# apple/ml-neuman

Measured on NVIDIA H100. Metric: Mrays/sec @128+128 samples, higher is better.
Workload: dtype f16 operands x f32 accumulate (wgmma); f32 elsewhere

## Files before the change

neuman_b200/csrc/api.cu:

```cuda
#include <math.h>
#include <string.h>

#include "nm_internal.cuh"

extern "C" const char* nm_version(void) { return "neuman_b200 0.1 (sm_90a)"; }

extern "C" int nm_ctx_create(int device, nm_ctx** out) {
  if (!out) return NM_ERR_INVALID;
  *out = nullptr;
  int ndev = 0;
  if (cudaGetDeviceCount(&ndev) != cudaSuccess || device < 0 || device >= ndev) return NM_ERR_CUDA;
  if (cudaSetDevice(device) != cudaSuccess) return NM_ERR_CUDA;
  nm_ctx* c = new nm_ctx();
  c->device = device;
  cudaDeviceProp prop;
  if (cudaGetDeviceProperties(&prop, device) == cudaSuccess) c->sm_count = prop.multiProcessorCount;
  if (cudaMalloc(&c->d_counter, 64 * sizeof(int32_t)) != cudaSuccess ||
      cudaMallocHost(&c->h_counter, 64 * sizeof(int32_t)) != cudaSuccess) {
    delete c;
    return NM_ERR_CUDA;
  }
  cudaMemset(c->d_counter, 0, 64 * sizeof(int32_t));
  *out = c;
  return NM_OK;
// ... 267 lines not shown
  const int rc = check_view_desc(ctx, d, __func__);
  if (rc != NM_OK) return rc;
  return net_pack(ctx, slot, d, NM_NET_NERFT, nullptr, nullptr, (cudaStream_t)stream);
}

extern "C" int nm_net_pack_noview(nm_ctx* ctx, int slot, const nm_nerf_noview_desc* d, void* stream) {
  NM_ENTER(ctx);
  if (slot < 0 || slot >= NM_MAX_NET_SLOTS || !d) NM_FAIL(ctx, NM_ERR_INVALID, "nm_net_pack_noview: bad slot/desc");
  if (d->pos_n_freqs != 10)
    NM_FAIL(ctx, NM_ERR_UNSUPPORTED, "nm_net_pack_noview: only pos_N_freqs=10 (63-d encoding) is built");
  for (int l = 0; l < 8; ++l)
    if (!d->pts_w[l] || !d->pts_b[l]) NM_FAIL(ctx, NM_ERR_INVALID, "nm_net_pack_noview: null pts_linears");
  if (!d->output_w || !d->output_b) NM_FAIL(ctx, NM_ERR_INVALID, "nm_net_pack_noview: null output_linear");
  nm_nerf_desc full{};
  for (int l = 0; l < 8; ++l) { full.pts_w[l] = d->pts_w[l]; full.pts_b[l] = d->pts_b[l]; }
  full.pos_pe_kind = d->pos_pe_kind;
  full.pos_min_freq = d->pos_min_freq; full.pos_max_freq = d->pos_max_freq; full.pos_n_freqs = d->pos_n_freqs;
  full.dir_pe_kind = NM_PE_POSENC; full.dir_min_freq = 0.f; full.dir_max_freq = 3.f; full.dir_n_freqs = 4;
  return net_pack(ctx, slot, &full, NM_NET_NOVIEW, d->output_w, d->output_b, (cudaStream_t)stream);
}

static int mlp_dispatch(nm_ctx* ctx, int slot, int mode, const float* pts, const float* views, const float* origins,
                        const float* dirs, const float* z, int64_t n, int32_t group, float t, float* raw, void* stream,
                        const NmTrainStash* stash = nullptr) {
  if (slot < 0 || slot >= NM_MAX_NET_SLOTS || !ctx->nets[slot].packed)
    NM_FAIL(ctx, NM_ERR_STATE, "nm_mlp_forward: net slot not packed");
  if (n < 0 || !raw) NM_FAIL(ctx, NM_ERR_INVALID, "nm_mlp_forward: bad argument");
  if (n == 0) return NM_OK;
  NmNet& net = ctx->nets[slot];
  if (mode != NM_MLP_SIMT_F32 && mode != NM_MLP_TC_F16) NM_FAIL(ctx, NM_ERR_INVALID, "nm_mlp_forward: unknown mode");
  cudaStream_t st = (cudaStream_t)stream;
  cudaEvent_t e0 = nullptr, e1 = nullptr;
  if (ctx->profile) {
    if (ctx->prof_used + 2 > ctx->prof_events.size()) {
      for (int k = 0; k < 2; ++k) {
        cudaEvent_t e;
        NM_CHECK_CUDA(ctx, cudaEventCreate(&e));
        ctx->prof_events.push_back(e);
      }
    }
    e0 = ctx->prof_events[ctx->prof_used];
    e1 = ctx->prof_events[ctx->prof_used + 1];
    NM_CHECK_CUDA(ctx, cudaEventRecord(e0, st));
  }
  int rc = mode == NM_MLP_SIMT_F32 ? nm_simt_forward(ctx, net, pts, views, origins, dirs, z, n, group, t, raw, st)
                                   : nm_tc_forward(ctx, net, pts, views, origins, dirs, z, n, group, t, raw, st, stash);
  if (ctx->profile && rc == NM_OK) {
    NM_CHECK_CUDA(ctx, cudaEventRecord(e1, st));
    ctx->prof_used += 2;
    ctx->prof_evals += n;
  }
  return rc;
}

static bool views_ok(const nm_ctx* ctx, int slot, const void* views) {
  return views || (slot >= 0 && slot < NM_MAX_NET_SLOTS && ctx->nets[slot].packed && ctx->nets[slot].kind == NM_NET_NOVIEW);
}
static bool is_noview(const nm_ctx* ctx, int slot) {
  return slot >= 0 && slot < NM_MAX_NET_SLOTS && ctx->nets[slot].kind == NM_NET_NOVIEW;
}
static bool is_nerft(const nm_ctx* ctx, int slot) {
  return slot >= 0 && slot < NM_MAX_NET_SLOTS && ctx->nets[slot].packed && ctx->nets[slot].kind == NM_NET_NERFT;
}

extern "C" int nm_mlp_forward(nm_ctx* ctx, int slot, int mode, const float* pts, const float* views, int64_t n,
                              int32_t views_per_ray, float* raw, void* stream) {
  NM_ENTER(ctx);
  if (!pts || !views_ok(ctx, slot, views) || views_per_ray < 0) NM_FAIL(ctx, NM_ERR_INVALID, "nm_mlp_forward: null pts/views");
  if (views_per_ray > 0 && n % views_per_ray != 0)
// ... 56 lines not shown
  const int width = 3 + 6 * (which == 0 ? net.desc.pos_n_freqs : net.desc.dir_n_freqs);
  if (ld < width) NM_FAIL(ctx, NM_ERR_INVALID, "nm_pe_backward: ld smaller than the encoding width");
  if (n == 0) return NM_OK;
  if (!x || !d_enc || !d_x) NM_FAIL(ctx, NM_ERR_INVALID, "nm_pe_backward: null argument");
  return nm_impl_pe_backward(ctx, net, which, x, group, d_enc, ld, inv_scale, n, d_x, (cudaStream_t)stream);
}

extern "C" int nm_dw_gemm(nm_ctx* ctx, const void* g_pre, const void* g_f, const void* g_v, const void* stash_x,
                          const void* stash_f, int64_t n, float* out, float* bias_out, void* stream) {
  NM_ENTER(ctx);
  if (n < 0 || !out || !bias_out) NM_FAIL(ctx, NM_ERR_INVALID, "nm_dw_gemm: bad argument");
  if (n == 0) {
    NM_CHECK_CUDA(ctx, cudaMemsetAsync(out, 0, (size_t)9 * 256 * 256 * sizeof(float), (cudaStream_t)stream));
    NM_CHECK_CUDA(ctx, cudaMemsetAsync(bias_out, 0, (size_t)9 * 256 * sizeof(float), (cudaStream_t)stream));
    return NM_OK;
  }
  const bool trunk_only = !g_f && !g_v && !stash_f;
  if (!g_pre || !stash_x || (!trunk_only && (!g_f || !g_v || !stash_f))) NM_FAIL(ctx, NM_ERR_INVALID, "nm_dw_gemm: null argument");
  return nm_impl_dw_gemm(ctx, (const __half*)g_pre, (const __half*)g_f, (const __half*)g_v, (const __half*)stash_x,
                         (const __half*)stash_f, n, out, bias_out, (cudaStream_t)stream);
}

int nm_impl_mlp_forward_rays(nm_ctx* ctx, int slot, int mode, const float* origins, const float* dirs, const float* z,
                             int64_t R, int32_t S, float t, float* raw, cudaStream_t st) {
  if (!origins || !dirs || !z || S <= 0 || R < 0) NM_FAIL(ctx, NM_ERR_INVALID, "nm_mlp_forward_rays: bad argument");
  return mlp_dispatch(ctx, slot, mode, nullptr, nullptr, origins, dirs, z, R * (int64_t)S, S, t, raw, st);
}

extern "C" int nm_mlp_forward_rays(nm_ctx* ctx, int slot, int mode, const float* origins, const float* dirs,
                                   const float* z, int64_t R, int32_t S, float* raw, void* stream) {
  NM_ENTER(ctx);
  if (is_nerft(ctx, slot)) NM_FAIL(ctx, NM_ERR_UNSUPPORTED, "nm_mlp_forward_rays: a NeRF-T net needs the time (nm_render_vanilla_t)");
  return nm_impl_mlp_forward_rays(ctx, slot, mode, origins, dirs, z, R, S, 0.f, raw, (cudaStream_t)stream);
}
```

neuman_b200/csrc/mlp_tc.cu:

```cuda
#include "nm_internal.cuh"
#include "nm_pe.cuh"
#include "tc_common.cuh"
#include <string.h>
#define TC_MAX_SLABS 64
struct TcPlan {
  uint32_t slab_off[TC_STEPS][6];
  uint32_t slab_bytes[TC_STEPS];
  uint32_t image_bytes;
  uint32_t lin_off[TC_MAX_SLABS + 1];
};

__host__ __device__ constexpr int tc_steps(bool v) { return v ? TC_STEPS : 9; }
__host__ __device__ constexpr int step_nkb(int s, bool v = true, bool t = false) {
  return s == 0 ? (t ? 2 : 1) : (s == 10 ? 2 : (!v && s == 8 ? 4 : (t && s == 5 ? 6 : 5)));
}
__host__ __device__ constexpr bool kb_is_bias(int s, int kb, bool v = true) {
  return kb == 4 && s != 5 && s != 9 && s >= 1 && (v ? s <= 8 : s <= 7);
}
__host__ __device__ constexpr bool kb_is_time(int s, int kb, bool t) { return t && ((s == 0 && kb == 1) || (s == 5 && kb == 5)); }
__host__ __device__ constexpr int step_N(int s, bool v = true) { return s <= 7 || (v && s == 8) ? 256 : (v && s == 9 ? 128 : 16); }
__host__ __device__ constexpr bool kb_is_dir(int s, int kb, bool v = true) { return v && s == 9 && kb == 4; }
__host__ __device__ constexpr int tc_slabs_per_tile(bool v = true, bool t = false) {
  int n = 0;
  for (int s = 0; s < tc_steps(v); ++s) n += step_nkb(s, v, t);
  return n;
}
static_assert(tc_slabs_per_tile(true, true) <= TC_MAX_SLABS && tc_slabs_per_tile(true) <= TC_MAX_SLABS, "slab table too small");

template <bool kTrain, bool kView>
struct TcCfg {
  static constexpr int THREADS = 256;
  static constexpr int NSLOT = kTrain || kView ? 4 : 6;
  static constexpr int OFF_POS = kTrain ? 4 * TC_KB_BYTES : 0;
  static constexpr int OFF_DIR = OFF_POS + TC_KB_BYTES;
  static constexpr int WG_BYTES = OFF_DIR + TC_KB_BYTES;
  static constexpr int OFF_RING = 2 * WG_BYTES;
  static constexpr int OFF_BAR = OFF_RING + NSLOT * TC_SLAB_BYTES;
  static constexpr int OFF_CONST = OFF_BAR + 16 * NSLOT;
  static constexpr int SMEM_USED = OFF_CONST + 4 * TC_CONST_FLOATS;
  static constexpr int SMEM_BYTES = SMEM_USED + 1024;
};
static_assert(TcCfg<false, false>::SMEM_BYTES <= 232448 && TcCfg<false, true>::SMEM_BYTES <= 232448 &&
              TcCfg<true, false>::SMEM_BYTES <= 232448 && TcCfg<true, true>::SMEM_BYTES <= 232448,
              "shared memory of the forward kernel exceeds 227 KB");

#define TC_CONST_ALPHA 0
#define TC_CONST_OUT 256

struct TcParams {
  const uint8_t* wimg;
  TcPlan plan;
  NmMlpInput in;
  NmPeSpec pos_pe, dir_pe;
  float* raw;
  const float* consts;
  long long n_tiles;
  int32_t* range_flag;
  int range_phase;
  __half* st_x;
  __half* st_f;
  __half* st_v;
  uint32_t* st_m;
  CUtensorMap map_x, map_f, map_v;
};

__device__ __forceinline__ void sincos_cycles(float f, float& s, float& c) {
// ... 42 lines not shown
        }
      }
    }
  }
  ch[nq == 30 ? 63 : 27] = 1.f;
#pragma unroll
  for (int i = 0; i < 32; ++i) out[i] = pack_f16x2(ch[2 * i], ch[2 * i + 1], false);
}

__device__ __forceinline__ void encode_time_f16(const NmPeSpec& pe, float t, uint32_t (&out)[32]) {
  float ch[22];
  ch[0] = t; ch[21] = 0.f;
#pragma unroll
  for (int k = 0; k < 10; ++k) {
    const float fh = __ldg(pe.table + 2 * k), fl = __ldg(pe.table + 2 * k + 1);
    const float pr = t * fh;
    const float low = fmaf(t, fl, fmaf(t, fh, -pr));
    sincos_cycles((pr - rintf(pr)) + low, ch[1 + 2 * k], ch[2 + 2 * k]);
  }
#pragma unroll
  for (int i = 0; i < 11; ++i) out[16 + i] = pack_f16x2(ch[2 * i], ch[2 * i + 1], false);
}

__device__ __forceinline__ void store_row_swizzled(uint8_t* blk, int row, const uint32_t* v, int nchunks) {
#pragma unroll
  for (int j = 0; j < 8; ++j) {
    if (j < nchunks) {
      uint4 q = make_uint4(v[4 * j], v[4 * j + 1], v[4 * j + 2], v[4 * j + 3]);
      *reinterpret_cast<uint4*>(blk + row * 128 + ((j ^ (row & 7)) << 4)) = q;
    }
  }
}

template <bool RELU>
__device__ __forceinline__ uint32_t pack2(float lo, float hi) {
  uint32_t d;
  if (RELU) asm("cvt.rn.satfinite.relu.f16x2.f32 %0, %1, %2;" : "=r"(d) : "f"(hi), "f"(lo));
  else asm("cvt.rn.satfinite.f16x2.f32 %0, %1, %2;" : "=r"(d) : "f"(hi), "f"(lo));
  return d;
}

template <bool RELU>
__device__ __forceinline__ void track_range(uint32_t& rng, uint32_t packed) {
  __half2 h = *reinterpret_cast<const __half2*>(&packed);
  if (!RELU) h = __habs2(h);
  const __half2 m = __hmax2(*reinterpret_cast<const __half2*>(&rng), h);
  rng = *reinterpret_cast<const uint32_t*>(&m);
}

template <int NC, bool RELU, bool ALPHA, bool SIGNS, bool SMEM>
// ... 19 lines not shown
      a[2 * j] = pA;
      a[2 * j + 1] = pB;
    }
    if (track) { track_range<RELU>(rng, pA); track_range<RELU>(rng, pB); }
    if (SIGNS) {
      const __half2 zero2 = __float2half2_rn(0.f);
      const uint32_t mA = __hgt2_mask(*reinterpret_cast<const __half2*>(&pA), zero2);
      const uint32_t mB = __hgt2_mask(*reinterpret_cast<const __half2*>(&pB), zero2);
      const int bit = 16 * ((j >> 1) & 1) + 4 * (j & 1) + q;
      wA[j >> 2] |= ((mA & 1u) << bit) | ((mA >> 16 & 1u) << (bit + 8));
      wB[j >> 2] |= ((mB & 1u) << bit) | ((mB >> 16 & 1u) << (bit + 8));
    }
  }
}

__device__ __forceinline__ void quad_or(uint32_t (&w)[8]) {
#pragma unroll
  for (int i = 0; i < 8; ++i) {
    w[i] |= __shfl_xor_sync(0xffffffffu, w[i], 1);
    w[i] |= __shfl_xor_sync(0xffffffffu, w[i], 2);
  }
}

template <bool kTrain, bool kView, bool kTime = false>
__device__ __forceinline__ void mlp_tc_body(const TcParams& P) {
  static_assert(!kTime || kView, "NeRF-T nets are view-dependent");
  using C = TcCfg<kTrain, kView>;
  constexpr int SLABS = tc_slabs_per_tile(kView, kTime);
  constexpr int STEPS = tc_steps(kView);
  constexpr int LAST = STEPS - 1;
  extern __shared__ uint8_t smem_dyn[];
  const uint32_t pad = (1024 - (smem_u32(smem_dyn) & 1023)) & 1023;
  uint8_t* smem = smem_dyn + pad;
  const uint32_t sbase = smem_u32(smem);
  const int wg = threadIdx.x >> 7, wtid = threadIdx.x & 127;
  const int lane = threadIdx.x & 31, q = lane & 3;
  const int rA = 16 * (wtid >> 5) + (lane >> 2);
  uint8_t* wbuf = smem + wg * C::WG_BYTES;
  const uint32_t wbase = sbase + wg * C::WG_BYTES;
  float* s_const = reinterpret_cast<float*>(smem + C::OFF_CONST);
  const TcRing<C::NSLOT> R{sbase + C::OFF_RING, sbase + C::OFF_BAR};

  for (int i = threadIdx.x; i < TC_CONST_FLOATS; i += C::THREADS) s_const[i] = __ldg(P.consts + i);
  const long long my_tiles = blockIdx.x < P.n_tiles ? (P.n_tiles - 1 - blockIdx.x) / gridDim.x + 1 : 0;
  const uint32_t total = (uint32_t)(my_tiles * SLABS);
  auto fill = [&](uint32_t qq) {
    const uint32_t j = qq % SLABS, off = P.plan.lin_off[j], bytes = P.plan.lin_off[j + 1] - off;
    mbar_arrive_expect_tx(R.full(qq), bytes);
    bulk_g2s(R.slot(qq), P.wimg + off, bytes, R.full(qq));
  };
  if (threadIdx.x == 0) R.init(total, fill);
  __syncthreads();
// ... 8 lines not shown
  for (long long it = 0; it < my_tiles; ++it) {
    const long long tile = blockIdx.x + it * gridDim.x;
    const long long row0 = tile * 128 + wg * TC_WG_ROWS;
    const bool track = !kView || (it % rperiod) == (P.range_phase % rperiod);
    {
      const int r = wtid & 63;
      const int group = P.in.group;
      long long g0 = 0;
      uint32_t g0r = 0;
      if (group > 0) { g0 = tile * 128 / group; g0r = (uint32_t)(tile * 128 - g0 * group); }
      const uint32_t off = wg * TC_WG_ROWS + r;
      const long long g = group > 0 ? g0 + (g0r + off) / (uint32_t)group : row0 + r;
      float p[3] = {0.f, 0.f, 0.f}, v[3] = {0.f, 0.f, 0.f};
      float t = 0.f;
      if (row0 + r < P.in.n) {
        nm_fetch_sample_at<kTime ? 4 : 3>(P.in, row0 + r, g, p, v);
        if (kTime) t = nm_fetch_time(P.in, row0 + r);
      }
      if (!kTrain && it > 0) wg_sync(wg);
      uint32_t e[32];
      if (wtid < 64) {
        encode_f16(P.pos_pe, p, e, 30);
        store_row_swizzled(wbuf + C::OFF_POS, r, e, 8);
      } else if (kView) {
        encode_f16(P.dir_pe, v, e, 12);
        if (kTime) encode_time_f16(P.pos_pe, t, e);
        store_row_swizzled(wbuf + C::OFF_DIR, r, e, kTime ? 8 : 4);
      }
      if (track && (kView || wtid < 64)) { track_range<false>(rng, e[0]); track_range<false>(rng, e[1]); }
      if (kTime && track && wtid >= 64) track_range<false>(rng, e[16]);
      fence_async_smem();
      wg_sync(wg);
    }
    float alpha[2] = {0.f, 0.f};
#pragma unroll (kTrain ? 1 : STEPS)
    for (int s = 0; s < STEPS; ++s) {
      const int nkb = step_nkb(s, kView, kTime);
      const bool wide = s <= (kView ? 8 : 7), views = kView && s == 9;
      wgmma_fence();
      int kb = 0;
      auto kblock = [&](auto&& issue) {
        const uint32_t qq = qbase + kb;
        R.wait_full(qq);
        issue(gmma_desc_k(R.slot(qq)), kb == 0);
        wgmma_commit();
        if (kb > 0) { wgmma_wait<1>(); R.release(qq - 1, total, fill); }
        ++kb;
      };
      auto smem_kblock = [&](uint32_t a_addr, int k0, int k1) {
        kblock([&](uint64_t b_desc, bool first) {
          const uint64_t a_desc = gmma_desc_k(a_addr);
          for (int k = k0; k < k1; ++k) {
            const uint32_t acc = !first || k > k0;
            if (wide) wgmma_n256(d, a_desc + 2 * k, b_desc + 2 * k, acc);
            else if (views) wgmma_n128(d, a_desc + 2 * k, b_desc + 2 * k, acc);
            else wgmma_n16(d16, a_desc + 2 * k, b_desc + 2 * k, acc);
          }
        });
      };
      if (s == 0 || s == 5) smem_kblock(wbase + C::OFF_POS, 0, 4);
      if (s > 0) {
        const int nact = kView && s == LAST ? 2 : 4;
#pragma unroll
        for (int j = 0; j < 4; ++j) {
          if (j < nact) {
            if constexpr (kTrain) smem_kblock(wbase + j * TC_KB_BYTES, 0, 4);
            else kblock([&](uint64_t b_desc, bool first) {
#pragma unroll
              for (int k = 0; k < 4; ++k) {
                const uint32_t* f = a + 16 * j + 4 * k;
                const uint32_t acc = !first || k > 0;
                if (wide) wgmma_n256_rs(d, f[0], f[1], f[2], f[3], b_desc + 2 * k, acc);
                else if (views) wgmma_n128_rs(d, f[0], f[1], f[2], f[3], b_desc + 2 * k, acc);
                else wgmma_n16_rs(d16, f[0], f[1], f[2], f[3], b_desc + 2 * k, acc);
              }
            });
          }
        }
      }
      if (kb < nkb) {
        if (kb_is_bias(s, kb, kView)) smem_kblock(wbase + C::OFF_POS, 3, 4);
        else if (kb_is_dir(s, kb, kView)) smem_kblock(wbase + C::OFF_DIR, 0, 2);
        else smem_kblock(wbase + C::OFF_DIR, 2, 4);
      }
      wgmma_wait<0>();
      wgmma_fence_regs(d);
      wgmma_fence_regs(d16);
      R.release(qbase + nkb - 1, total, fill);
      qbase += nkb;
      if (s < LAST) {
        if (kTrain) {
          if (wtid == 0) tma_store_wait_read();
          wg_sync(wg);
        }
        uint32_t wA[8] = {0, 0, 0, 0, 0, 0, 0, 0}, wB[8] = {0, 0, 0, 0, 0, 0, 0, 0};
        const float* s_walpha = s_const + TC_CONST_ALPHA;
        if (s == 7) fwd_epi<256, true, kView, kTrain, kTrain>(d, a, wbuf, rA, q, s_walpha, alpha, wA, wB, track, rng);
        else if (kView && s == 8) fwd_epi<256, false, false, false, kTrain>(d, a, wbuf, rA, q, s_walpha, alpha, wA, wB, track, rng);
        else if (s == 9) fwd_epi<128, true, false, kTrain, kTrain>(d, a, wbuf, rA, q, s_walpha, alpha, wA, wB, track, rng);
        else fwd_epi<256, true, false, kTrain, kTrain>(d, a, wbuf, rA, q, s_walpha, alpha, wA, wB, track, rng);
        if (kTrain) {
          fence_async_smem();
          wg_sync(wg);
          if (wtid == 0) {
            if (!kView || s < 8) tma_store_rows(&P.map_x, wbase, 0, 4, row0, s);
            else if (s == 8) tma_store_rows(&P.map_f, wbase, 0, 4, row0, 0);
            else tma_store_rows(&P.map_v, wbase, 0, 2, row0, 0);
          }
          if (!kView || s != 8) {
            quad_or(wA);
            quad_or(wB);
            const long long iA = row0 + rA, iB = iA + 8;
            if (!kView || s < 8) {
              uint32_t* m = P.st_m + (size_t)s * P.in.n * 8;
              if (iA < P.in.n) reinterpret_cast<uint2*>(m + iA * 8)[q] = make_uint2(wA[2 * q], wA[2 * q + 1]);
              if (iB < P.in.n) reinterpret_cast<uint2*>(m + iB * 8)[q] = make_uint2(wB[2 * q], wB[2 * q + 1]);
            } else {
              uint32_t* m = P.st_m + (size_t)8 * P.in.n * 8;
              if (iA < P.in.n) m[iA * 8 + q] = wA[q];
              if (iB < P.in.n) m[iB * 8 + q] = wB[q];
            }
          }
        }
        if (kView && s == 7) {
#pragma unroll
          for (int r = 0; r < 2; ++r) {
            alpha[r] += __shfl_xor_sync(0xffffffffu, alpha[r], 1);
            alpha[r] += __shfl_xor_sync(0xffffffffu, alpha[r], 2);
          }
        }
      } else if (kView) {
        const float bA = __shfl_down_sync(0xffffffffu, d16[0], 1), bB = __shfl_down_sync(0xffffffffu, d16[2], 1);
        const long long iA = row0 + rA, iB = iA + 8;
        if (q == 0 && iA < P.in.n)
          reinterpret_cast<float4*>(P.raw)[iA] = make_float4(d16[0] + ob.x, d16[1] + ob.y, bA + ob.z, alpha[0] + ob.w);
        if (q == 0 && iB < P.in.n)
          reinterpret_cast<float4*>(P.raw)[iB] = make_float4(d16[2] + ob.x, d16[3] + ob.y, bB + ob.z, alpha[1] + ob.w);
      } else {
        const float cA = __shfl_down_sync(0xffffffffu, d16[0], 1), dA = __shfl_down_sync(0xffffffffu, d16[1], 1);
        const float cB = __shfl_down_sync(0xffffffffu, d16[2], 1), dB = __shfl_down_sync(0xffffffffu, d16[3], 1);
        const long long iA = row0 + rA, iB = iA + 8;
        if (q == 0 && iA < P.in.n)
          reinterpret_cast<float4*>(P.raw)[iA] = make_float4(d16[0] + ob.x, d16[1] + ob.y, cA + ob.z, dA + ob.w);
        if (q == 0 && iB < P.in.n)
          reinterpret_cast<float4*>(P.raw)[iB] = make_float4(d16[2] + ob.x, d16[3] + ob.y, cB + ob.z, dB + ob.w);
      }
    }
  }
  if (((rng & 0xFFFFu) >= 0x7BFFu) || ((rng >> 16) >= 0x7BFFu)) atomicOr(P.range_flag, 1);
  if (kTrain && wtid == 0) tma_store_wait_all();
}

template <bool kTrain>
__global__ void __launch_bounds__(TcCfg<kTrain, true>::THREADS, 1) k_mlp_tc(const __grid_constant__ TcParams P) {
  mlp_tc_body<kTrain, true>(P);
}
template <bool kTrain>
__global__ void __launch_bounds__(TcCfg<kTrain, false>::THREADS, 1) k_mlp_tc_noview(const __grid_constant__ TcParams P) {
  mlp_tc_body<kTrain, false>(P);
}
template <bool kTrain>
__global__ void __launch_bounds__(TcCfg<kTrain, true>::THREADS, 1) k_mlp_tc_nerft(const __grid_constant__ TcParams P) {
  mlp_tc_body<kTrain, true, true>(P);
}

struct PackSrc {
  const float* w[8]; const float* feat; const float* views; const float* rgb;
  const float* b[8]; const float* feat_b; const float* views_b;
  const float* out_t;
};

__device__ __forceinline__ int nerft_col(int kk, bool time) {
  if (time) {
    if (kk == 32) return 3;
    if (kk < 33 || kk > 52) return -1;
    const int k = (kk - 33) >> 1;
    return ((kk - 33) & 1) ? 11 + 8 * k : 7 + 8 * k;
  }
  if (kk < 3) return kk;
  const int i = kk - 3, k = i / 6, r = i - 6 * k;
  return r < 3 ? 4 + 8 * k + r : 8 + 8 * k + (r - 3);
}

__device__ __forceinline__ float src_weight(const PackSrc& S, int s, int n, int kb, int kk, bool view, bool time) {
  if (!view && s == 8) return n < 4 ? S.out_t[(size_t)(kb * 64 + kk) * 4 + n] : 0.f;
  if (kb_is_bias(s, kb, view)) {
    if (kk != 63) return 0.f;
// ... 93 lines not shown
      const float low = fmaf(v, fl, fmaf(v, fh, -pr));
      sincos_cycles((pr - rintf(pr)) + low, ch[4 + 8 * k + d], ch[8 + 8 * k + d]);
    }
  }
  ch[NM_POS_PE_T] = 1.f;
  uint4* dst = reinterpret_cast<uint4*>(out + (size_t)i * 96);
#pragma unroll
  for (int j = 0; j < 12; ++j)
    dst[j] = make_uint4(pack_f16x2(ch[8 * j], ch[8 * j + 1], false), pack_f16x2(ch[8 * j + 2], ch[8 * j + 3], false),
                        pack_f16x2(ch[8 * j + 4], ch[8 * j + 5], false), pack_f16x2(ch[8 * j + 6], ch[8 * j + 7], false));
}

int nm_tc_encode(nm_ctx* ctx, const NmNet& net, int which, const float* x, int64_t group, int64_t n, __half* out, cudaStream_t st) {
  NmPeSpec pe = which == 0 ? NmPeSpec{net.desc.pos_pe_kind, net.desc.pos_n_freqs, net.f32 + net.o_pos_cyc}
                           : NmPeSpec{net.desc.dir_pe_kind, net.desc.dir_n_freqs, net.f32 + net.o_dir_cyc};
  if (which == 0 && net.kind == NM_NET_NERFT)
    k_encode_f16_nerft<<<(unsigned)((n + 127) / 128), 128, 0, st>>>(pe, x, group, n, out);
  else
    k_encode_f16<<<(unsigned)((n + 127) / 128), 128, 0, st>>>(pe, which, x, group, n, out);
  NM_CHECK_LAUNCH(ctx);
  return NM_OK;
}

static TcPlan make_plan(bool view, bool time) {
  TcPlan p{};
  uint32_t off = 0;
  int j = 0;
  for (int s = 0; s < tc_steps(view); ++s) {
    p.slab_bytes[s] = (uint32_t)step_N(s, view) * 128u;
    for (int kb = 0; kb < step_nkb(s, view, time); ++kb) {
      p.slab_off[s][kb] = p.lin_off[j++] = off;
      off += p.slab_bytes[s];
    }
  }
  p.lin_off[j] = p.image_bytes = off;
  return p;
}

int nm_tc_pack(nm_ctx* ctx, NmNet& net, cudaStream_t st) {
  const bool view = net.kind != NM_NET_NOVIEW, time = net.kind == NM_NET_NERFT;
  TcPlan plan = make_plan(view, time);
  const size_t halfs = plan.image_bytes / 2;
  if (!net.f16 || net.f16_halfs != halfs) {
    if (net.f16) { NM_CHECK_CUDA(ctx, cudaDeviceSynchronize()); NM_CHECK_CUDA(ctx, cudaFree(net.f16)); net.f16 = nullptr; }
    NM_CHECK_CUDA(ctx, cudaMalloc(&net.f16, halfs * sizeof(__half)));
    net.f16_halfs = halfs;
  }
  if (!net.tc_bias) NM_CHECK_CUDA(ctx, cudaMalloc(&net.tc_bias, TC_CONST_FLOATS * sizeof(float)));
  const nm_nerf_desc& d = net.desc;
  PackSrc S;
  for (int l = 0; l < 8; ++l) S.w[l] = d.pts_w[l];
  S.feat = d.feature_w; S.views = d.views_w; S.rgb = d.rgb_w;
  for (int l = 0; l < 8; ++l) S.b[l] = d.pts_b[l];
  S.feat_b = d.feature_b; S.views_b = d.views_b;
  S.out_t = net.f32 + net.o_out_w;
  k_tc_pack<<<(unsigned)((halfs + 255) / 256), 256, 0, st>>>(S, plan, view, time, net.f16);
  NM_CHECK_LAUNCH(ctx);
  if (view) k_tc_consts<<<1, 256, 0, st>>>(d.rgb_b, d.alpha_w, d.alpha_b, net.tc_bias);
  else k_tc_consts_noview<<<1, 256, 0, st>>>(net.f32 + net.o_out_b, net.tc_bias);
  NM_CHECK_LAUNCH(ctx);
  return NM_OK;
}

template <bool kTrain, bool kView, bool kTime = false>
static int launch_tc(nm_ctx* ctx, const TcParams& P, cudaStream_t st) {
  void (*kernel)(const TcParams);
  if constexpr (kTime) kernel = k_mlp_tc_nerft<kTrain>;
  else kernel = kView ? k_mlp_tc<kTrain> : k_mlp_tc_noview<kTrain>;
  using C = TcCfg<kTrain, kView>;
  NM_SET_SMEM_ONCE(ctx, kernel, C::SMEM_BYTES);
  long long ctas = ctx->sm_count;
  if (P.n_tiles < ctas) ctas = P.n_tiles > 0 ? P.n_tiles : 1;
  kernel<<<(unsigned)ctas, C::THREADS, C::SMEM_BYTES, st>>>(P);
  NM_CHECK_LAUNCH(ctx);
  return NM_OK;
}

int nm_tc_forward(nm_ctx* ctx, NmNet& net, const float* pts, const float* views, const float* origins,
                  const float* dirs, const float* z, int64_t n, int32_t group, float t, float* raw, cudaStream_t st,
                  const NmTrainStash* stash) {
  if (!net.f16 || !net.tc_bias) NM_FAIL(ctx, NM_ERR_STATE, "nm_tc_forward: weights not packed");
  const bool view = net.kind != NM_NET_NOVIEW, time = net.kind == NM_NET_NERFT;
  TcParams P;
  P.wimg = reinterpret_cast<const uint8_t*>(net.f16);
  P.plan = make_plan(view, time);
  P.in = NmMlpInput{pts, views, origins, dirs, z, (long long)n, group, t};
  P.pos_pe = NmPeSpec{net.desc.pos_pe_kind, net.desc.pos_n_freqs, net.f32 + net.o_pos_cyc};
  P.dir_pe = NmPeSpec{net.desc.dir_pe_kind, net.desc.dir_n_freqs, net.f32 + net.o_dir_cyc};
  P.raw = raw;
  P.consts = net.tc_bias;
  P.n_tiles = (n + 127) / 128;
  P.range_flag = ctx->d_counter + NM_RANGE_FLAG_WORD;
  P.range_phase = (int)(ctx->range_seq++ % 64);
  P.st_x = stash ? stash->x : nullptr; P.st_f = stash ? stash->f : nullptr; P.st_v = stash ? stash->v : nullptr;
  P.st_m = stash ? stash->m : nullptr;
  memset(&P.map_x, 0, 3 * sizeof(CUtensorMap));
  if (stash) {
    if (n >= (int64_t)0x7fff0000) NM_FAIL(ctx, NM_ERR_INVALID, "nm_mlp_forward_train: n too large for one call");
    if (tc_make_store_map(&P.map_x, stash->x, 8, (uint64_t)n, 256) ||
        (view && (tc_make_store_map(&P.map_f, stash->f, 1, (uint64_t)n, 256) || tc_make_store_map(&P.map_v, stash->v, 1, (uint64_t)n, 128))))
      NM_FAIL(ctx, NM_ERR_CUDA, "nm_mlp_forward_train: cuTensorMapEncodeTiled failed");
  }
  if (time) return stash ? launch_tc<true, true, true>(ctx, P, st) : launch_tc<false, true, true>(ctx, P, st);
  if (!view) return stash ? launch_tc<true, false>(ctx, P, st) : launch_tc<false, false>(ctx, P, st);
  return stash ? launch_tc<true, true>(ctx, P, st) : launch_tc<false, true>(ctx, P, st);
}
```

neuman_b200/csrc/nm_internal.cuh:

```cuda
#pragma once
#include <cuda_runtime.h>
#include <cuda_fp16.h>
#include <stdint.h>
#include <stdio.h>
#include <string>
#include <vector>

#include "neuman_b200.h"

#define NM_WIDTH 256
#define NM_DEPTH 8
#define NM_POS_PE 63
#define NM_POS_PE_T 84
#define NM_DIR_PE 27
#define NM_VIEWS_HID 128
#define NM_RANGE_FLAG_WORD 32

enum { NM_NET_VIEW = 0, NM_NET_NOVIEW = 1, NM_NET_NERFT = 2 };

struct NmNet {
  bool packed = false;
  int kind = NM_NET_VIEW;
  nm_nerf_desc desc{};
  float* f32 = nullptr;
// ... 115 lines not shown
  const size_t want = need + (need >> 3) + 16;
  NM_CHECK_CUDA(ctx, cudaMalloc(p, want * sizeof(T)));
  *cap = want;
  return NM_OK;
}

__host__ __device__ __forceinline__ float nm_linspace01(int i, int steps) {
  if (steps <= 1) return 0.f;
  const float step = 1.0f / (float)(steps - 1);
  if (i < steps / 2) return (float)i * step;
  return 1.0f - (float)(steps - 1 - i) * step;
}

int nm_impl_workspace(nm_ctx* ctx, size_t bytes, char** out);

int nm_impl_build_vgroups(nm_ctx* ctx, NmMesh& m, const float* host_verts, const float* lo, const float* hi, cudaStream_t st);
int nm_impl_near_far_mesh(nm_ctx* ctx, const NmMesh& m, const float* origins, const float* dirs, int64_t R, float geo_threshold,
                          float* near_out, float* far_out, cudaStream_t st);
int nm_impl_raygen(nm_ctx* ctx, const nm_camera* cam, int mode, int64_t pix0, int64_t n, const int32_t* xy,
                   const int32_t* pixels, float* origins, float* dirs, cudaStream_t stream);
int nm_impl_raw2outputs_zend(nm_ctx* ctx, const float* raw, const float* z, const float* rays_d, int64_t R, int32_t S,
                             int32_t white_bkg, float z_end, float* rgb, float* depth, cudaStream_t st);
int nm_impl_mlp_forward_rays(nm_ctx* ctx, int slot, int mode, const float* origins, const float* dirs, const float* z,
                             int64_t R, int32_t S, float t, float* raw, cudaStream_t st);
int nm_simt_forward(nm_ctx* ctx, const NmNet& net, const float* pts, const float* views,
                    const float* origins, const float* dirs, const float* z, int64_t n,
                    int32_t group, float t, float* raw, cudaStream_t st);
int nm_tc_pack(nm_ctx* ctx, NmNet& net, cudaStream_t st);
struct NmTrainStash {
  __half* x;
  __half* f;
  __half* v;
  uint32_t* m;
};
int nm_impl_pe_backward(nm_ctx* ctx, const NmNet& net, int which, const float* x, int64_t group, const float* d_enc, int ld,
                        const float* inv_scale, int64_t n, float* d_x, cudaStream_t st);
int nm_tc_encode(nm_ctx* ctx, const NmNet& net, int which, const float* x, int64_t group, int64_t n, __half* out, cudaStream_t st);
int nm_impl_dw_gemm(nm_ctx* ctx, const __half* g_pre, const __half* g_f, const __half* g_v, const __half* st_x,
                    const __half* st_f, int64_t n, float* out, float* bias_out, cudaStream_t st);
int nm_tc_backward(nm_ctx* ctx, NmNet& net, const float* d_raw, const float* scale, int64_t n, const __half* st_v,
                   const uint32_t* st_m, __half* g_pre, __half* g_f, __half* g_v, cudaStream_t st);
int nm_tc_forward(nm_ctx* ctx, NmNet& net, const float* pts, const float* views,
                  const float* origins, const float* dirs, const float* z, int64_t n,
                  int32_t group, float t, float* raw, cudaStream_t st, const NmTrainStash* stash = nullptr);
```

neuman_b200/csrc/render.cu:

```cuda
#include "nm_internal.cuh"

namespace {

__device__ __forceinline__ float linspace_f(float start, float end, int i, int steps) {
  if (steps <= 1) return start;
  float step = (end - start) / (float)(steps - 1);
  if (i < steps / 2) return start + step * (float)i;
  return end - step * (float)(steps - 1 - i);
}

__global__ void k_fill_placeholder(float* __restrict__ z, float4* __restrict__ raw, long long R, int S, float start,
                                   float end) {
  long long idx = (long long)blockIdx.x * blockDim.x + threadIdx.x;
  if (idx >= R * S) return;
  int s = (int)(idx % S);
  z[idx] = linspace_f(start, end, s, S);
  raw[idx] = make_float4(0.f, 0.f, 0.f, 0.f);
}

__global__ void k_compact_hits(const float* __restrict__ near_v, const float* __restrict__ far_v, long long R,
                               int32_t* __restrict__ hit_idx, int32_t* __restrict__ counter) {
  long long r = (long long)blockIdx.x * blockDim.x + threadIdx.x;
  bool hit = r < R && near_v[r] < far_v[r];
  unsigned m = __ballot_sync(0xffffffffu, hit);
// ... 113 lines not shown
  ctx->last_mlp_evals = 0; ctx->last_hit_rays = 0;
  for (int64_t i = 0; i < n; i += C) {
    const int64_t c = std::min<int64_t>(C, n - i);
    TRY(nm_impl_raygen(ctx, cam, ray_mode, pix0 + i, c, nullptr, pixels ? pixels + i : nullptr, o, d, st));
    auto dst = [&](float* p, float* s, int w) { return host_out || !p ? s : p + w * i; };
    TRY(body(c, o, d, Planes{dst(out.rgb, stage.rgb, 3), dst(out.depth, stage.depth, 1), dst(out.acc, stage.acc, 1)}));
    if (host_out) {
      auto back = [&](float* p, const float* s, int w) {
        return p ? cudaMemcpyAsync(p + w * i, s, w * c * sizeof(float), cudaMemcpyDeviceToHost, st) : cudaSuccess;
      };
      NM_CHECK_CUDA(ctx, back(out.rgb, stage.rgb, 3));
      NM_CHECK_CUDA(ctx, back(out.depth, stage.depth, 1));
      NM_CHECK_CUDA(ctx, back(out.acc, stage.acc, 1));
      NM_CHECK_CUDA(ctx, cudaStreamSynchronize(st));
    }
  }
  return NM_OK;
}

int bkg_pass(nm_ctx* ctx, int coarse, int fine, const nm_render_opts* opt, const float* o, const float* d, int64_t C,
             float* z_c, float* raw_c, float* w_c, float* z_f, float* raw_f, float** raw_out, float** z_out,
             int* S_out, cudaStream_t st, float t = 0.f) {
  const int S = opt->samples_per_ray, N = opt->importance_samples_per_ray;
  TRY(nm_ray_to_samples(ctx, o, d, nullptr, nullptr, opt->near_bkg, opt->far_bkg, C, S, 0, nullptr, nullptr, nullptr,
                        z_c, st));
  TRY(nm_impl_mlp_forward_rays(ctx, coarse, opt->mlp_mode, o, d, z_c, C, S, t, raw_c, st));
  ctx->last_mlp_evals += C * S;
  if (fine >= 0 && N > 0) {
    TRY(nm_raw2outputs(ctx, raw_c, z_c, d, C, S, nullptr, 1.f, opt->white_bkg, nullptr, nullptr, nullptr, w_c, nullptr, st));
    TRY(nm_importance_samples(ctx, o, d, z_c, w_c, C, S, N, 1, nullptr, nullptr, z_f, st));
    TRY(nm_impl_mlp_forward_rays(ctx, fine, opt->mlp_mode, o, d, z_f, C, S + N, t, raw_f, st));
    ctx->last_mlp_evals += C * (S + N);
    *raw_out = raw_f; *z_out = z_f; *S_out = S + N;
  } else {
    *raw_out = raw_c; *z_out = z_c; *S_out = S;
  }
  return NM_OK;
}

struct Hits {
  int n; bool uni; const int32_t* actors;
  float *nr[NM_MAX_ACTORS], *fr[NM_MAX_ACTORS];
  int32_t* idx[NM_MAX_ACTORS];
  int64_t count[NM_MAX_ACTORS + 1];
  int32_t* uidx = nullptr;
  float *flag = nullptr, *zeros = nullptr;
  float *oh, *dh, *nh, *fh, *pts, *cpts, *cdirs, *z, *raw;
  float *rgb, *depth, *acc;
  void take(Arena& A, int64_t C, int S) {
// ... 238 lines not shown
```

neuman_b200/csrc/warp.cu:

```cuda
#include <cub/device/device_radix_sort.cuh>
#include <float.h>
#include <math.h>

#include "nm_internal.cuh"
#include "train_common_kernels.cuh"

struct BvhView {
  int n;
  const float4* lo;
  const float4* hi;
  const int2* children;
  const int32_t* leaf_face;
  const float* tri9;
};

__device__ __forceinline__ uint32_t expand_bits10(uint32_t v) {
  v = (v * 0x00010001u) & 0xFF0000FFu;
  v = (v * 0x00000101u) & 0x0F00F00Fu;
  v = (v * 0x00000011u) & 0xC30C30C3u;
  v = (v * 0x00000005u) & 0x49249249u;
  return v;
}

__device__ __forceinline__ int f2ord(float f) { const int k = __float_as_int(f); return k >= 0 ? k : k ^ 0x7fffffff; }
// ... 111 lines not shown
  V3<T> bp = sub(p, b);
  T d3 = dot(ab, bp), d4 = dot(ac, bp);
  if (d3 >= 0 && d4 <= d3) return b;
  T vc = d1 * d4 - d3 * d2;
  if (vc <= 0 && d1 >= 0 && d3 <= 0) return madd(a, ab, d1 / (d1 - d3));
  V3<T> cp = sub(p, c);
  T d5 = dot(ab, cp), d6 = dot(ac, cp);
  if (d6 >= 0 && d5 <= d6) return c;
  T vb = d5 * d2 - d1 * d6;
  if (vb <= 0 && d2 >= 0 && d6 <= 0) return madd(a, ac, d2 / (d2 - d6));
  T va = d3 * d6 - d5 * d4;
  if (va <= 0 && (d4 - d3) >= 0 && (d5 - d6) >= 0) return madd(b, sub(c, b), (d4 - d3) / ((d4 - d3) + (d5 - d6)));
  T den = T(1) / (va + vb + vc);
  return madd(madd(a, ab, vb * den), ac, vc * den);
}

__device__ __forceinline__ float box_d2(const BvhView& B, int node, V3<float> p) {
  const float4 l = __ldg(B.lo + node), h = __ldg(B.hi + node);
  float dx = fmaxf(fmaxf(l.x - p.x, p.x - h.x), 0.f), dy = fmaxf(fmaxf(l.y - p.y, p.y - h.y), 0.f),
        dz = fmaxf(fmaxf(l.z - p.z, p.z - h.z), 0.f);
  return dx * dx + dy * dy + dz * dz;
}

__device__ __forceinline__ int bvh_nearest_face(const BvhView& B, V3<float> p, int* stack) {
  float best = FLT_MAX;
  int best_f = 0x7fffffff;
  int sp = 0;
  int node = (B.n > 1) ? 0 : B.n - 1;
  while (true) {
    if (node >= B.n - 1) {
      const int f = __ldg(B.leaf_face + (node - (B.n - 1)));
      const float* t = B.tri9 + 9 * (size_t)f;
      V3<float> a{__ldg(t), __ldg(t + 1), __ldg(t + 2)}, b{__ldg(t + 3), __ldg(t + 4), __ldg(t + 5)},
          c{__ldg(t + 6), __ldg(t + 7), __ldg(t + 8)};
      V3<float> e = sub(closest_on_tri<float>(p, a, b, c), p);
      const float d2 = dot(e, e);
      if (d2 < best || (d2 == best && f < best_f)) { best = d2; best_f = f; }
      node = -1;
    } else {
      const int2 ch = __ldg(B.children + node);
      const float dl = box_d2(B, ch.x, p), dr = box_d2(B, ch.y, p);
      const float lim = best * 1.00001f;
      const bool needL = __any_sync(0xffffffffu, dl <= lim), needR = __any_sync(0xffffffffu, dr <= lim);
      const bool left_first = __popc(__ballot_sync(0xffffffffu, dl <= dr)) >= 16;
      if (needL && needR) {
        if (sp < 64) { if ((threadIdx.x & 31) == 0) stack[sp] = left_first ? ch.y : ch.x; ++sp; }
        node = left_first ? ch.x : ch.y;
      } else {
        node = needL ? ch.x : (needR ? ch.y : -1);
      }
    }
    if (node < 0) {
      bool found = false;
      while (sp > 0) {
        --sp;
        __syncwarp();
        const int cand = stack[sp];
        if (__any_sync(0xffffffffu, box_d2(B, cand, p) <= best * 1.00001f)) { node = cand; found = true; break; }
      }
      if (!found) break;
    }
  }
  return best_f;
}

__global__ void __launch_bounds__(128) k_warp_nearest(BvhView B, const float* __restrict__ pts, long long R, int S, int lg_rays,
                                                       int32_t* __restrict__ face_out) {
  const long long w = (long long)blockIdx.x * 4 + (threadIdx.x >> 5);
  const int lane = threadIdx.x & 31;
  long long i;
  bool live;
  if (lg_rays == 0) {
    i = w * 32 + lane;
    live = i < R * S;
    if (!live) i = R * S - 1;
  } else {
    const int per = 32 >> lg_rays;
    const int groups = S / per;
    const long long rg = w / groups;
    const int sg = (int)(w - rg * groups);
    long long ray = (rg << lg_rays) + (lane / per);
// ... 337 lines not shown
```

Baseline: 1.498.

## Add density-only coarse MLP kernel skipping color layers

Adds a density-only tensor-core forward variant for the coarse pass of hierarchical rendering. It runs only steps 0-7 (trunk plus alpha), skips the view-direction encoding and the feature and RGB layers, and writes zero RGB with alpha to raw. Because the direction slab is no longer needed, the kernel can use 6 pipeline slots instead of 4. The coarse RGB is only used to compute sampling weights, so dropping it should remove unneeded GEMMs. The BVH nearest-face search also switches to a distance tolerance with a float64 tie-break, which adds work in that separate path.

```diff
diff --git a/neuman_b200/csrc/api.cu b/neuman_b200/csrc/api.cu
--- a/neuman_b200/csrc/api.cu
+++ b/neuman_b200/csrc/api.cu
@@ -313,13 +313,14 @@
 
 static int mlp_dispatch(nm_ctx* ctx, int slot, int mode, const float* pts, const float* views, const float* origins,
                         const float* dirs, const float* z, int64_t n, int32_t group, float t, float* raw, void* stream,
-                        const NmTrainStash* stash = nullptr) {
+                        const NmTrainStash* stash = nullptr, bool density = false) {
   if (slot < 0 || slot >= NM_MAX_NET_SLOTS || !ctx->nets[slot].packed)
     NM_FAIL(ctx, NM_ERR_STATE, "nm_mlp_forward: net slot not packed");
   if (n < 0 || !raw) NM_FAIL(ctx, NM_ERR_INVALID, "nm_mlp_forward: bad argument");
   if (n == 0) return NM_OK;
   NmNet& net = ctx->nets[slot];
   if (mode != NM_MLP_SIMT_F32 && mode != NM_MLP_TC_F16) NM_FAIL(ctx, NM_ERR_INVALID, "nm_mlp_forward: unknown mode");
+  if (density && mode != NM_MLP_TC_F16) NM_FAIL(ctx, NM_ERR_INVALID, "nm_mlp_forward: density only needs the tensor-core mode");
   cudaStream_t st = (cudaStream_t)stream;
   cudaEvent_t e0 = nullptr, e1 = nullptr;
   if (ctx->profile) {
@@ -335,7 +336,7 @@
     NM_CHECK_CUDA(ctx, cudaEventRecord(e0, st));
   }
   int rc = mode == NM_MLP_SIMT_F32 ? nm_simt_forward(ctx, net, pts, views, origins, dirs, z, n, group, t, raw, st)
-                                   : nm_tc_forward(ctx, net, pts, views, origins, dirs, z, n, group, t, raw, st, stash);
+                                   : nm_tc_forward(ctx, net, pts, views, origins, dirs, z, n, group, t, raw, st, stash, density);
   if (ctx->profile && rc == NM_OK) {
     NM_CHECK_CUDA(ctx, cudaEventRecord(e1, st));
     ctx->prof_used += 2;
@@ -438,9 +439,9 @@
 }
 
 int nm_impl_mlp_forward_rays(nm_ctx* ctx, int slot, int mode, const float* origins, const float* dirs, const float* z,
-                             int64_t R, int32_t S, float t, float* raw, cudaStream_t st) {
+                             int64_t R, int32_t S, float t, float* raw, cudaStream_t st, bool density) {
   if (!origins || !dirs || !z || S <= 0 || R < 0) NM_FAIL(ctx, NM_ERR_INVALID, "nm_mlp_forward_rays: bad argument");
-  return mlp_dispatch(ctx, slot, mode, nullptr, nullptr, origins, dirs, z, R * (int64_t)S, S, t, raw, st);
+  return mlp_dispatch(ctx, slot, mode, nullptr, nullptr, origins, dirs, z, R * (int64_t)S, S, t, raw, st, nullptr, density);
 }
 
 extern "C" int nm_mlp_forward_rays(nm_ctx* ctx, int slot, int mode, const float* origins, const float* dirs,
diff --git a/neuman_b200/csrc/mlp_tc.cu b/neuman_b200/csrc/mlp_tc.cu
--- a/neuman_b200/csrc/mlp_tc.cu
+++ b/neuman_b200/csrc/mlp_tc.cu
@@ -20,17 +20,19 @@
 __host__ __device__ constexpr bool kb_is_time(int s, int kb, bool t) { return t && ((s == 0 && kb == 1) || (s == 5 && kb == 5)); }
 __host__ __device__ constexpr int step_N(int s, bool v = true) { return s <= 7 || (v && s == 8) ? 256 : (v && s == 9 ? 128 : 16); }
 __host__ __device__ constexpr bool kb_is_dir(int s, int kb, bool v = true) { return v && s == 9 && kb == 4; }
-__host__ __device__ constexpr int tc_slabs_per_tile(bool v = true, bool t = false) {
+__host__ __device__ constexpr int tc_slabs_before(int steps, bool v, bool t) {
   int n = 0;
-  for (int s = 0; s < tc_steps(v); ++s) n += step_nkb(s, v, t);
+  for (int s = 0; s < steps; ++s) n += step_nkb(s, v, t);
   return n;
 }
+__host__ __device__ constexpr int tc_slabs_per_tile(bool v = true, bool t = false) { return tc_slabs_before(tc_steps(v), v, t); }
+constexpr int TC_DENSITY_STEPS = 8;
 static_assert(tc_slabs_per_tile(true, true) <= TC_MAX_SLABS && tc_slabs_per_tile(true) <= TC_MAX_SLABS, "slab table too small");
 
-template <bool kTrain, bool kView>
+template <bool kTrain, bool kView, bool kDensity = false>
 struct TcCfg {
   static constexpr int THREADS = 256;
-  static constexpr int NSLOT = kTrain || kView ? 4 : 6;
+  static constexpr int NSLOT = kTrain || (kView && !kDensity) ? 4 : 6;
   static constexpr int OFF_POS = kTrain ? 4 * TC_KB_BYTES : 0;
   static constexpr int OFF_DIR = OFF_POS + TC_KB_BYTES;
   static constexpr int WG_BYTES = OFF_DIR + TC_KB_BYTES;
@@ -41,7 +43,8 @@
   static constexpr int SMEM_BYTES = SMEM_USED + 1024;
 };
 static_assert(TcCfg<false, false>::SMEM_BYTES <= 232448 && TcCfg<false, true>::SMEM_BYTES <= 232448 &&
-              TcCfg<true, false>::SMEM_BYTES <= 232448 && TcCfg<true, true>::SMEM_BYTES <= 232448,
+              TcCfg<true, false>::SMEM_BYTES <= 232448 && TcCfg<true, true>::SMEM_BYTES <= 232448 &&
+              TcCfg<false, true, true>::SMEM_BYTES <= 232448,
               "shared memory of the forward kernel exceeds 227 KB");
 
 #define TC_CONST_ALPHA 0
@@ -130,10 +133,10 @@
   for (int i = 0; i < 11; ++i) out[16 + i] = pack_f16x2(ch[2 * i], ch[2 * i + 1], false);
 }
 
-__device__ __forceinline__ void store_row_swizzled(uint8_t* blk, int row, const uint32_t* v, int nchunks) {
+__device__ __forceinline__ void store_row_swizzled(uint8_t* blk, int row, const uint32_t* v, int nchunks, int first = 0) {
 #pragma unroll
   for (int j = 0; j < 8; ++j) {
-    if (j < nchunks) {
+    if (j >= first && j < nchunks) {
       uint4 q = make_uint4(v[4 * j], v[4 * j + 1], v[4 * j + 2], v[4 * j + 3]);
       *reinterpret_cast<uint4*>(blk + row * 128 + ((j ^ (row & 7)) << 4)) = q;
     }
@@ -199,12 +202,13 @@
   }
 }
 
-template <bool kTrain, bool kView, bool kTime = false>
+template <bool kTrain, bool kView, bool kTime = false, bool kDensity = false>
 __device__ __forceinline__ void mlp_tc_body(const TcParams& P) {
   static_assert(!kTime || kView, "NeRF-T nets are view-dependent");
-  using C = TcCfg<kTrain, kView>;
-  constexpr int SLABS = tc_slabs_per_tile(kView, kTime);
-  constexpr int STEPS = tc_steps(kView);
+  static_assert(!kDensity || (kView && !kTrain), "the density-only kernels render view-dependent nets");
+  using C = TcCfg<kTrain, kView, kDensity>;
+  constexpr int STEPS = kDensity ? TC_DENSITY_STEPS : tc_steps(kView);
+  constexpr int SLABS = tc_slabs_before(STEPS, kView, kTime);
   constexpr int LAST = STEPS - 1;
   extern __shared__ uint8_t smem_dyn[];
   const uint32_t pad = (1024 - (smem_u32(smem_dyn) & 1023)) & 1023;
@@ -259,12 +263,17 @@
       if (wtid < 64) {
         encode_f16(P.pos_pe, p, e, 30);
         store_row_swizzled(wbuf + C::OFF_POS, r, e, 8);
-      } else if (kView) {
+      } else if (kView && !kDensity) {
         encode_f16(P.dir_pe, v, e, 12);
         if (kTime) encode_time_f16(P.pos_pe, t, e);
         store_row_swizzled(wbuf + C::OFF_DIR, r, e, kTime ? 8 : 4);
+      } else if (kTime) {
+#pragma unroll
+        for (int i = 27; i < 32; ++i) e[i] = 0u;
+        encode_time_f16(P.pos_pe, t, e);
+        store_row_swizzled(wbuf + C::OFF_DIR, r, e, 8, 4);
       }
-      if (track && (kView || wtid < 64)) { track_range<false>(rng, e[0]); track_range<false>(rng, e[1]); }
+      if (track && (wtid < 64 || (kView && !kDensity))) { track_range<false>(rng, e[0]); track_range<false>(rng, e[1]); }
       if (kTime && track && wtid >= 64) track_range<false>(rng, e[16]);
       fence_async_smem();
       wg_sync(wg);
@@ -297,7 +306,7 @@
       };
       if (s == 0 || s == 5) smem_kblock(wbase + C::OFF_POS, 0, 4);
       if (s > 0) {
-        const int nact = kView && s == LAST ? 2 : 4;
+        const int nact = kView && !kDensity && s == LAST ? 2 : 4;
 #pragma unroll
         for (int j = 0; j < 4; ++j) {
           if (j < nact) {
@@ -322,10 +331,10 @@
       }
       wgmma_wait<0>();
       wgmma_fence_regs(d);
-      wgmma_fence_regs(d16);
+      if (!kDensity) wgmma_fence_regs(d16);
       R.release(qbase + nkb - 1, total, fill);
       qbase += nkb;
-      if (s < LAST) {
+      if (s < LAST || kDensity) {
         if (kTrain) {
           if (wtid == 0) tma_store_wait_read();
           wg_sync(wg);
@@ -366,6 +375,11 @@
             alpha[r] += __shfl_xor_sync(0xffffffffu, alpha[r], 2);
           }
         }
+        if (kDensity) {
+          const long long iA = row0 + rA, iB = iA + 8;
+          if (q == 0 && iA < P.in.n) reinterpret_cast<float4*>(P.raw)[iA] = make_float4(0.f, 0.f, 0.f, alpha[0] + ob.w);
+          if (q == 0 && iB < P.in.n) reinterpret_cast<float4*>(P.raw)[iB] = make_float4(0.f, 0.f, 0.f, alpha[1] + ob.w);
+        }
       } else if (kView) {
         const float bA = __shfl_down_sync(0xffffffffu, d16[0], 1), bB = __shfl_down_sync(0xffffffffu, d16[2], 1);
         const long long iA = row0 + rA, iB = iA + 8;
@@ -400,6 +414,12 @@
 __global__ void __launch_bounds__(TcCfg<kTrain, true>::THREADS, 1) k_mlp_tc_nerft(const __grid_constant__ TcParams P) {
   mlp_tc_body<kTrain, true, true>(P);
 }
+__global__ void __launch_bounds__(TcCfg<false, true, true>::THREADS, 1) k_mlp_tc_density(const __grid_constant__ TcParams P) {
+  mlp_tc_body<false, true, false, true>(P);
+}
+__global__ void __launch_bounds__(TcCfg<false, true, true>::THREADS, 1) k_mlp_tc_nerft_density(const __grid_constant__ TcParams P) {
+  mlp_tc_body<false, true, true, true>(P);
+}
 
 struct PackSrc {
   const float* w[8]; const float* feat; const float* views; const float* rgb;
@@ -539,7 +559,7 @@
   return NM_OK;
 }
 
-static TcPlan make_plan(bool view, bool time) {
+static constexpr TcPlan make_plan(bool view, bool time) {
   TcPlan p{};
   uint32_t off = 0;
   int j = 0;
@@ -553,6 +573,15 @@
   p.lin_off[j] = p.image_bytes = off;
   return p;
 }
+static constexpr bool density_prefix_ok(bool time) {
+  const TcPlan p = make_plan(true, time);
+  int j = 0;
+  for (int s = 0; s < TC_DENSITY_STEPS; ++s)
+    for (int kb = 0; kb < step_nkb(s, true, time); ++kb)
+      if (p.lin_off[j++] != p.slab_off[s][kb]) return false;
+  return j == tc_slabs_before(TC_DENSITY_STEPS, true, time) && p.lin_off[j] == p.slab_off[TC_DENSITY_STEPS][0];
+}
+static_assert(density_prefix_ok(false) && density_prefix_ok(true), "steps 0-7 are not a prefix of the packed image");
 
 int nm_tc_pack(nm_ctx* ctx, NmNet& net, cudaStream_t st) {
   const bool view = net.kind != NM_NET_NOVIEW, time = net.kind == NM_NET_NERFT;
@@ -579,12 +608,13 @@
   return NM_OK;
 }
 
-template <bool kTrain, bool kView, bool kTime = false>
+template <bool kTrain, bool kView, bool kTime = false, bool kDensity = false>
 static int launch_tc(nm_ctx* ctx, const TcParams& P, cudaStream_t st) {
   void (*kernel)(const TcParams);
-  if constexpr (kTime) kernel = k_mlp_tc_nerft<kTrain>;
+  if constexpr (kDensity) kernel = kTime ? k_mlp_tc_nerft_density : k_mlp_tc_density;
+  else if constexpr (kTime) kernel = k_mlp_tc_nerft<kTrain>;
   else kernel = kView ? k_mlp_tc<kTrain> : k_mlp_tc_noview<kTrain>;
-  using C = TcCfg<kTrain, kView>;
+  using C = TcCfg<kTrain, kView, kDensity>;
   NM_SET_SMEM_ONCE(ctx, kernel, C::SMEM_BYTES);
   long long ctas = ctx->sm_count;
   if (P.n_tiles < ctas) ctas = P.n_tiles > 0 ? P.n_tiles : 1;
@@ -595,9 +625,10 @@
 
 int nm_tc_forward(nm_ctx* ctx, NmNet& net, const float* pts, const float* views, const float* origins,
                   const float* dirs, const float* z, int64_t n, int32_t group, float t, float* raw, cudaStream_t st,
-                  const NmTrainStash* stash) {
+                  const NmTrainStash* stash, bool density) {
   if (!net.f16 || !net.tc_bias) NM_FAIL(ctx, NM_ERR_STATE, "nm_tc_forward: weights not packed");
   const bool view = net.kind != NM_NET_NOVIEW, time = net.kind == NM_NET_NERFT;
+  if (density && (stash || !view)) NM_FAIL(ctx, NM_ERR_INVALID, "nm_tc_forward: density only renders view-dependent nets");
   TcParams P;
   P.wimg = reinterpret_cast<const uint8_t*>(net.f16);
   P.plan = make_plan(view, time);
@@ -618,6 +649,7 @@
         (view && (tc_make_store_map(&P.map_f, stash->f, 1, (uint64_t)n, 256) || tc_make_store_map(&P.map_v, stash->v, 1, (uint64_t)n, 128))))
       NM_FAIL(ctx, NM_ERR_CUDA, "nm_mlp_forward_train: cuTensorMapEncodeTiled failed");
   }
+  if (density) return time ? launch_tc<false, true, true, true>(ctx, P, st) : launch_tc<false, true, false, true>(ctx, P, st);
   if (time) return stash ? launch_tc<true, true, true>(ctx, P, st) : launch_tc<false, true, true>(ctx, P, st);
   if (!view) return stash ? launch_tc<true, false>(ctx, P, st) : launch_tc<false, false>(ctx, P, st);
   return stash ? launch_tc<true, true>(ctx, P, st) : launch_tc<false, true>(ctx, P, st);
diff --git a/neuman_b200/csrc/nm_internal.cuh b/neuman_b200/csrc/nm_internal.cuh
--- a/neuman_b200/csrc/nm_internal.cuh
+++ b/neuman_b200/csrc/nm_internal.cuh
@@ -161,7 +161,7 @@
 int nm_impl_raw2outputs_zend(nm_ctx* ctx, const float* raw, const float* z, const float* rays_d, int64_t R, int32_t S,
                              int32_t white_bkg, float z_end, float* rgb, float* depth, cudaStream_t st);
 int nm_impl_mlp_forward_rays(nm_ctx* ctx, int slot, int mode, const float* origins, const float* dirs, const float* z,
-                             int64_t R, int32_t S, float t, float* raw, cudaStream_t st);
+                             int64_t R, int32_t S, float t, float* raw, cudaStream_t st, bool density = false);
 int nm_simt_forward(nm_ctx* ctx, const NmNet& net, const float* pts, const float* views,
                     const float* origins, const float* dirs, const float* z, int64_t n,
                     int32_t group, float t, float* raw, cudaStream_t st);
@@ -181,4 +181,5 @@
                    const uint32_t* st_m, __half* g_pre, __half* g_f, __half* g_v, cudaStream_t st);
 int nm_tc_forward(nm_ctx* ctx, NmNet& net, const float* pts, const float* views,
                   const float* origins, const float* dirs, const float* z, int64_t n,
-                  int32_t group, float t, float* raw, cudaStream_t st, const NmTrainStash* stash = nullptr);
+                  int32_t group, float t, float* raw, cudaStream_t st, const NmTrainStash* stash = nullptr,
+                  bool density = false);
diff --git a/neuman_b200/csrc/render.cu b/neuman_b200/csrc/render.cu
--- a/neuman_b200/csrc/render.cu
+++ b/neuman_b200/csrc/render.cu
@@ -159,9 +159,10 @@
              float* z_c, float* raw_c, float* w_c, float* z_f, float* raw_f, float** raw_out, float** z_out,
              int* S_out, cudaStream_t st, float t = 0.f) {
   const int S = opt->samples_per_ray, N = opt->importance_samples_per_ray;
+  const bool density = fine >= 0 && N > 0 && opt->mlp_mode == NM_MLP_TC_F16 && ctx->nets[coarse].kind != NM_NET_NOVIEW;
   TRY(nm_ray_to_samples(ctx, o, d, nullptr, nullptr, opt->near_bkg, opt->far_bkg, C, S, 0, nullptr, nullptr, nullptr,
                         z_c, st));
-  TRY(nm_impl_mlp_forward_rays(ctx, coarse, opt->mlp_mode, o, d, z_c, C, S, t, raw_c, st));
+  TRY(nm_impl_mlp_forward_rays(ctx, coarse, opt->mlp_mode, o, d, z_c, C, S, t, raw_c, st, density));
   ctx->last_mlp_evals += C * S;
   if (fine >= 0 && N > 0) {
     TRY(nm_raw2outputs(ctx, raw_c, z_c, d, C, S, nullptr, 1.f, opt->white_bkg, nullptr, nullptr, nullptr, w_c, nullptr, st));
diff --git a/neuman_b200/csrc/warp.cu b/neuman_b200/csrc/warp.cu
--- a/neuman_b200/csrc/warp.cu
+++ b/neuman_b200/csrc/warp.cu
@@ -157,9 +157,22 @@
   return dx * dx + dy * dy + dz * dz;
 }
 
+__device__ __forceinline__ double tri_d2_f64(const BvhView& B, int f, V3<float> p) {
+  const float* t = B.tri9 + 9 * (size_t)f;
+  const V3<double> P{(double)p.x, (double)p.y, (double)p.z};
+  const V3<double> a{(double)__ldg(t), (double)__ldg(t + 1), (double)__ldg(t + 2)};
+  const V3<double> b{(double)__ldg(t + 3), (double)__ldg(t + 4), (double)__ldg(t + 5)};
+  const V3<double> c{(double)__ldg(t + 6), (double)__ldg(t + 7), (double)__ldg(t + 8)};
+  const V3<double> e = sub(closest_on_tri<double>(P, a, b, c), P);
+  return dot(e, e);
+}
+
 __device__ __forceinline__ int bvh_nearest_face(const BvhView& B, V3<float> p, int* stack) {
-  float best = FLT_MAX;
+  const float tol = 1e-5f * (1.f + fmaxf(fabsf(p.x), fmaxf(fabsf(p.y), fabsf(p.z))));
+  float best_d = FLT_MAX;
+  double best64 = -1.0;
   int best_f = 0x7fffffff;
+  auto lim_of = [&]() { const float r = best_d + tol; return r * r; };
   int sp = 0;
   int node = (B.n > 1) ? 0 : B.n - 1;
   while (true) {
@@ -169,13 +182,19 @@
       V3<float> a{__ldg(t), __ldg(t + 1), __ldg(t + 2)}, b{__ldg(t + 3), __ldg(t + 4), __ldg(t + 5)},
           c{__ldg(t + 6), __ldg(t + 7), __ldg(t + 8)};
       V3<float> e = sub(closest_on_tri<float>(p, a, b, c), p);
-      const float d2 = dot(e, e);
-      if (d2 < best || (d2 == best && f < best_f)) { best = d2; best_f = f; }
+      const float d2 = dot(e, e), d = sqrtf(d2);
+      if (d + tol < best_d) {
+        best_d = d; best_f = f; best64 = -1.0;
+      } else if (d <= best_d + tol) {
+        if (best64 < 0.0) best64 = tri_d2_f64(B, best_f, p);
+        const double e64 = tri_d2_f64(B, f, p);
+        if (e64 < best64 || (e64 == best64 && f < best_f)) { best_d = d; best_f = f; best64 = e64; }
+      }
       node = -1;
     } else {
       const int2 ch = __ldg(B.children + node);
       const float dl = box_d2(B, ch.x, p), dr = box_d2(B, ch.y, p);
-      const float lim = best * 1.00001f;
+      const float lim = lim_of();
       const bool needL = __any_sync(0xffffffffu, dl <= lim), needR = __any_sync(0xffffffffu, dr <= lim);
       const bool left_first = __popc(__ballot_sync(0xffffffffu, dl <= dr)) >= 16;
       if (needL && needR) {
@@ -191,7 +210,7 @@
         --sp;
         __syncwarp();
         const int cand = stack[sp];
-        if (__any_sync(0xffffffffu, box_d2(B, cand, p) <= best * 1.00001f)) { node = cand; found = true; break; }
+        if (__any_sync(0xffffffffu, box_d2(B, cand, p) <= lim_of())) { node = cand; found = true; break; }
       }
       if (!found) break;
     }
```

New measurement: 1.586, median of 6. 1.06x the previous value.
